# wdc3iii/legged_gym_dev

Hardware: AMD Instinct MI355X
Metric: env-steps/sec (whole node), ANYmal-C flat 4096 envs per GPU (higher is better)
Workload: dtype f32

## Files before the change

### legged_gym_dev_amd/csrc/ppo_api.hip

```cpp
#include <cstdlib>
#include <cstring>
#include <string>
#include <vector>

#include "ppo_device.h"
#include "ppo_mlp_args.h"
#include "ppo_rnn.h"

void lg_set_error(const std::string &s);

extern "C" {
void ppok_gemm_fwd(const GemmArgs *g, int nz, hipStream_t s);
void ppok_gemm_dx(const GemmArgs *g, int nz, hipStream_t s);
void ppok_sync_planes(const PpoDev *P, hipStream_t s);
int ppok_mlp_fwd(const MlpArgs *g, const PpoDev *P, hipStream_t s);
int ppok_mlp_supported(const MlpArgs *g);
int64_t ppok_mlp_frag_elems(int K, int N);
void ppok_mlp_frag_build(const MlpArgs *g, hipStream_t s);
void ppok_gemm_dw(const GemmArgs *g, int nz, hipStream_t s);
void ppok_act_sample(const PpoDev *P, const float *obs, const float *cobs, const float *mu, const float *val, int t,
                     int64_t cnt, int inject, hipStream_t s);
void ppok_process_step(const PpoDev *P, const float *rew, const uint8_t *dones, const uint8_t *tos, int t, hipStream_t s);
void ppok_gae(const PpoDev *P, const float *last_values, hipStream_t s);
void ppok_det_fold(const PpoDev *P, hipStream_t s);
void ppok_adv_normalize(const PpoDev *P, hipStream_t s);
void ppok_gather(const PpoDev *P, int mb, hipStream_t s);
void ppok_randperm(const PpoDev *P, int n, uint64_t update_idx, hipStream_t s);
void ppok_loss(const PpoDev *P, const float *mu, const float *v, float *dmu, float *dval, hipStream_t s);
// ... 61 lines not shown
    hipEvent_t ev_dz, ev_side;
    int overlap;
    long long *det_buf;
    int act_code;
    int grads_dirty;
    lg_ctx *env;
    int pp_pending, pp_t, pp_use_tos;
    int params_dirty;
    int fused_act;
    MlpArgs mlp;
    int step, inject;
    int64_t act_count, update_count;
    int Mmax;
    std::vector<void *> allocs;
    int64_t perm_count;
    struct MbSet { float *obs, *critic_obs, *actions, *mu, *scalars; } mbset[2];
    int mb_cur, mb_ready, mb_last;
    lg_ppo_buffers pub;
    Rnn rnn;
};

template <typename T>
static bool palloc(lg_ppo *p, T **out, size_t n) {
    void *q = nullptr;
    size_t bytes = (n ? n : 1) * sizeof(T);
    if (hipMalloc(&q, bytes) != hipSuccess || hipMemset(q, 0, bytes) != hipSuccess) return false;
    p->allocs.push_back(q);
    *out = (T *)q;
    return true;
}
#define PA(ptr, n) do { if (!palloc(p, &(ptr), (n))) { lg_set_error("hipMalloc failed in lg_ppo_create"); lg_ppo_destroy(p); return -100; } } while (0)
// ... 51 lines not shown
    int64_t counts[4];
    const int n = bucket_extents(p, l, bufs, counts);
    hipStream_t cs = lg_comm_stream_(p->comm);
    (void)hipEventRecord(p->ev_bucket, ready_on);
    (void)hipStreamWaitEvent(cs, p->ev_bucket, 0);
    const int rc = lg_comm_group_allreduce_(p->comm, bufs, counts, n, cs);
    if (rc && !p->comm_rc) p->comm_rc = rc;
}

static void backward(lg_ppo *p, int M, const float *in0, const float *in1, int skip_head = 0) {
    const float *in[2] = {in0, in1};
    auto det_args = [&](GemmArgs &g) {
        g.det_base = p->dev.grads; g.det64 = p->dev.det64; g.det_n = p->dev.num_params + 2;
    };
    const int nl = p->net[0].nl;
    for (int l = nl - 1 - skip_head; l >= 0; --l) {
        GemmArgs g;
        memset(&g, 0, sizeof(g));
        det_args(g);
        for (int z = 0; z < 2; ++z) {
            Net &n = p->net[z];
            g.A[z] = n.dz[l + 1]; g.lda[z] = n.dims[l + 1];
            g.B[z] = l == 0 ? in[z] : n.act[l]; g.ldb[z] = n.dims[l];
            g.C[z] = p->dev.grads + n.w_off[l]; g.ldc[z] = n.dims[l];
            g.M[z] = n.dims[l + 1]; g.N[z] = n.dims[l]; g.K[z] = M;
            if (l == 0 && !p->rnn.H) {
                const int ldp = z == 0 ? p->dev.Op : p->dev.OCp;
                g.ldb[z] = ldp;
                if (ldp != n.dims[0]) { g.N[z] = ldp; g.nstore[z] = n.dims[0]; }
            }
        }
        const bool on_side = p->overlap && l > 0;
        hipStream_t dw_stream = on_side ? p->side : p->stream;
        if (on_side) {
// ... 5 lines not shown
        if (l > 0) {
            memset(&g, 0, sizeof(g));
            det_args(g);
            for (int z = 0; z < 2; ++z) {
                Net &n = p->net[z];
                g.A[z] = n.dz[l + 1]; g.lda[z] = n.dims[l + 1];
                g.B[z] = p->dev.params + n.w_off[l]; g.ldb[z] = n.dims[l];
                g.Bpl[z] = p->dev.wpl + n.pl_off[l];
                g.C[z] = n.dz[l]; g.ldc[z] = n.dims[l];
                g.aux[z] = n.act[l]; g.ldaux[z] = n.dims[l];
                g.colsum[z] = p->dev.grads + n.b_off[l - 1];
                g.M[z] = M; g.N[z] = n.dims[l]; g.K[z] = n.dims[l + 1];
            }
            g.elu = p->act_code;
            g.pl_stride = p->dev.pl_stride;
            ppok_gemm_dx(&g, 2, p->stream);
        }
    }
    if (p->rnn.H) {
        GemmArgs g;
        memset(&g, 0, sizeof(g));
        for (int z = 0; z < 2; ++z) {
            Net &n = p->net[z];
            g.A[z] = n.dz[1]; g.lda[z] = n.dims[1];
            g.B[z] = p->dev.params + n.w_off[0]; g.ldb[z] = n.dims[0];
            g.Bpl[z] = p->dev.wpl + n.pl_off[0];
            g.C[z] = p->rnn.dh[z]; g.ldc[z] = n.dims[0];
            g.aux[z] = p->rnn.dh[z]; g.ldaux[z] = n.dims[0];
            g.M[z] = M; g.N[z] = n.dims[0]; g.K[z] = n.dims[1];
        }
        g.elu = 0;
// ... 272 lines not shown
                dest[d.seg_off[sg] + e] = (int32_t)(d.seg_pl[sg] + (e / d.seg_cols[sg]) * seg_ld[sg] + e % d.seg_cols[sg]);
        (void)hipMemcpy(d.pl_dest, dest.data(), dest.size() * sizeof(int32_t), hipMemcpyHostToDevice);
    }
    const size_t TN = (size_t)T * N;
    PA(d.st_obs, TN * O);
    if (cfg->num_critic_obs > 0) PA(d.st_critic_obs, TN * OC); else d.st_critic_obs = d.st_obs;
    PA(d.st_actions, TN * A); PA(d.st_rewards, TN); PA(d.st_values, TN); PA(d.st_returns, TN); PA(d.st_adv, TN);
    PA(d.st_log_prob, TN); PA(d.st_mu, TN * A); PA(d.st_sigma, A); PA(d.st_dones, TN);
    PA(d.act_actions, (size_t)N * A); PA(d.act_values, N); PA(d.act_log_prob, N); PA(d.act_mu, (size_t)N * A);
    PA(d.stats, 8); PA(d.loss_acc, 4 + LG_NORM_BLOCKS); PA(d.noise, (size_t)N * A); PA(d.perm, TN); PA(d.adv_partial, 4);
    for (int k = 0; k < 2; ++k) {
        lg_ppo::MbSet &m = p->mbset[k];
        PA(m.obs, (size_t)R * d.Op);
        if (cfg->num_critic_obs > 0) PA(m.critic_obs, (size_t)R * d.OCp); else m.critic_obs = m.obs;
        PA(m.actions, (size_t)R * A); PA(m.mu, (size_t)R * A); PA(m.scalars, (size_t)R * 4);
    }
    p->mb_cur = 0; p->mb_ready = -1; p->mb_last = -1;
    d.mb_obs = p->mbset[0].obs; d.mb_critic_obs = p->mbset[0].critic_obs; d.mb_actions = p->mbset[0].actions;
    d.mb_mu = p->mbset[0].mu; d.mb_scalars = p->mbset[0].scalars;
    PA(d.head_part, ppok_head_part_floats());
    PA(d.cur_reward_sum, N); PA(d.cur_episode_len, N); PA(d.ep_stats, 4); PA(d.ep_ring, 200); PA(d.ep_ring_count, 1);
    for (int z = 0; z < 2; ++z) {
        Net &n = p->net[z];
        n.act[0] = nullptr; n.dz[0] = nullptr;
        for (int l = 1; l <= n.nl; ++l) { PA(n.act[l], (size_t)p->Mmax * n.dims[l]); PA(n.dz[l], (size_t)p->Mmax * n.dims[l]); }
    }
    if (H) {
        Rnn &q = p->rnn;
        const size_t NH = (size_t)N * H, Rr = (size_t)R;
        for (int z = 0; z < 2; ++z) {
            PA(q.h[z], NH); PA(q.c[z], NH); PA(q.sv_h[z], TN * H); PA(q.sv_c[z], TN * H); PA(q.tmp_h[z], NH); PA(q.tmp_c[z], NH);
            PA(q.pg[z], Rr * 4 * H); PA(q.gates[z], Rr * 4 * H);
            PA(q.hout[z], Rr * H); PA(q.cout[z], Rr * H); PA(q.hused[z], Rr * H); PA(q.cused[z], Rr * H); PA(q.dh[z], Rr * H);
            PA(q.dc[z], (size_t)q.mbs * H);
// ... 57 lines not shown
    return 0;
}
int lg_ppo_reset_hidden(lg_ppo *p, const uint8_t *dones) {
    if (!p->rnn.H) { lg_set_error("lg_ppo_reset_hidden: not a recurrent learner"); return -15; }
    flush_rollout_epilogue(p);
    const Rnn &q = p->rnn;
    ppok_lstm_reset(q.h[0], q.c[0], q.h[1], q.c[1], dones, p->cfg.num_envs, q.H, p->stream);
    return launch_ok();
}
int lg_ppo_get_buffers(lg_ppo *p, lg_ppo_buffers *out) { *out = p->pub; return 0; }
int lg_ppo_set_stream(lg_ppo *p, void *s) { p->stream = (hipStream_t)s; return 0; }
int lg_ppo_inject_noise(lg_ppo *p, int enable) { p->inject = enable; return 0; }
int lg_ppo_debug_set_overlap(lg_ppo *p, int v) { p->overlap = v; return 0; }
int lg_ppo_debug_set_fused_act(lg_ppo *p, int v) { p->fused_act = v && p->mlp.wfrag; return 0; }
int lg_ppo_debug_get_fused_act(lg_ppo *p) { return p->fused_act; }
int lg_ppo_debug_set_act_count(lg_ppo *p, long long v) { p->act_count = v; return 0; }

int lg_ppo_param_layout(lg_ppo *p, int64_t *offsets, int64_t *shapes, int max_entries) {
    int k = 0;
    auto put = [&](int64_t o, int64_t r, int64_t c) {
        if (k < max_entries) { offsets[k] = o; shapes[2 * k] = r; shapes[2 * k + 1] = c; }
        ++k;
    };
    put(p->dev.off_std, p->cfg.num_actions, 0);
    for (int z = 0; z < 2; ++z)
        for (int l = 0; l < p->net[z].nl; ++l) {
            put(p->net[z].w_off[l], p->net[z].dims[l + 1], p->net[z].dims[l]);
            put(p->net[z].b_off[l], p->net[z].dims[l + 1], 0);
        }
    const Rnn &q = p->rnn;
// ... 119 lines not shown
    p->grads_dirty = 1;
    ppok_sync_planes(&p->dev, p->stream);
    return launch_ok();
}

int lg_ppo_minibatch_backward(lg_ppo *p, int epoch, int mb) {
    (void)epoch;
    if (rnn_update_refused(p)) return -6;
    PpoDev &d = p->dev;
    const int R = d.mb_rows;
    if (p->grads_dirty) (void)hipMemsetAsync(d.grads, 0, (size_t)(d.num_params + 2) * sizeof(float), p->stream);
    p->grads_dirty = 1;
    auto use_set = [&](PpoDev &dev, int k) {
        const lg_ppo::MbSet &m = p->mbset[k];
        dev.mb_obs = m.obs; dev.mb_critic_obs = m.critic_obs; dev.mb_actions = m.actions; dev.mb_mu = m.mu; dev.mb_scalars = m.scalars;
    };
    if (p->mb_ready == mb) {
        p->mb_cur ^= 1;
        use_set(d, p->mb_cur);
    } else {
        ppok_gather(&d, mb, p->stream);
    }
    p->mb_ready = -1;
    p->mb_last = mb;
    Net &na = p->net[0], &nc = p->net[1];
    const int nl = na.nl, H3 = na.dims[nl - 1];
    const bool fuse = p->act_code == 1 && nl >= 2 && nc.dims[nl - 1] == H3 && (H3 == 128 || H3 == 64 || H3 == 32);
    if (p->rnn.H) {
        rnn_forward_seq(p, mb);
        forward(p, R, p->rnn.hout[0], p->rnn.hout[1], 3, fuse ? 1 : 0, true, false);
// ... 11 lines not shown
        rnn_backward_seq(p, mb);
    } else
        backward(p, R, d.mb_obs, d.mb_critic_obs, fuse ? 1 : 0);
    if (d.det64) ppok_det_fold(&d, p->stream);
    if (p->comm_rc) { const int rc = p->comm_rc; p->comm_rc = 0; return rc; }
    return launch_ok();
}

int lg_ppo_minibatch_step(lg_ppo *p) {
    int next = -1;
    PpoDev other = p->dev;
    if (p->cfg.num_mini_batches > 1 && p->mb_last >= 0) {
        next = (p->mb_last + 1) % p->cfg.num_mini_batches;
        const lg_ppo::MbSet &m = p->mbset[p->mb_cur ^ 1];
        other.mb_obs = m.obs; other.mb_critic_obs = m.critic_obs; other.mb_actions = m.actions; other.mb_mu = m.mu; other.mb_scalars = m.scalars;
    }
    if (ppok_step(&p->dev, (int)(p->update_count & 1), &other, next, p->stream)) p->mb_ready = next;
    p->mb_last = -1;
    p->grads_dirty = 0;
    p->params_dirty = 1;
    p->update_count++;
    return launch_ok();
}

int lg_ppo_end_update(lg_ppo *p) { p->step = 0; return 0; }

int lg_ppo_set_comm(lg_ppo *p, lg_comm *c) {
    if (c && p->rnn.H) { lg_set_error("lg_ppo_set_comm: the per-layer gradient buckets do not cover the LSTM of a recurrent learner; reduce the whole gradient buffer between lg_ppo_minibatch_backward and lg_ppo_minibatch_step instead"); return -14; }
    if (c && p->dev.det64) { lg_set_error("gradient buckets inside the backward pass cannot be combined with deterministic mode"); return -14; }
    p->comm = c;
// ... 41 lines not shown
    const int n = bucket_extents(p, l, bufs, counts);
    for (int k = 0; k < n; ++k) offsets[k] = bufs[k] - p->dev.grads;
    return n;
}

int lg_ppo_debug_mb_sets(lg_ppo *p, void **cur, void **other, int *dims) {
    const PpoDev &d = p->dev;
    const lg_ppo::MbSet &m = p->mbset[p->mb_cur ^ 1];
    void *c[5] = {d.mb_obs, d.mb_critic_obs, d.mb_actions, d.mb_mu, d.mb_scalars};
    void *o[5] = {m.obs, m.critic_obs, m.actions, m.mu, m.scalars};
    for (int k = 0; k < 5; ++k) { cur[k] = c[k]; other[k] = o[k]; }
    dims[0] = d.Op; dims[1] = d.OCp; dims[2] = d.mb_rows;
    return 0;
}

int lg_ppo_debug_weight_planes(lg_ppo *p, void **wpl, int64_t *pl_stride, void **pl_dest) {
    if (!p || !wpl || !pl_stride || !pl_dest) { lg_set_error("null argument"); return -1; }
    *wpl = p->dev.wpl; *pl_stride = p->dev.pl_stride; *pl_dest = p->dev.pl_dest;
    return 0;
}

int lg_ppo_act_inference(lg_ppo *p, const float *obs, float *actions_out, int64_t rows) {
    if (rows > p->Mmax) { lg_set_error("too many rows for act_inference"); return -11; }
    if (p->rnn.H) {
        if (rows != p->cfg.num_envs) { lg_set_error("act_inference of a recurrent learner takes exactly num_envs rows"); return -11; }
        rnn_stash_live(p, 1, -1);
        rnn_live_step(p, 1, obs, nullptr, -1);
        obs = p->rnn.h[0];
    }
    forward(p, (int)rows, obs, nullptr, 1);
// ... 8 lines not shown
```

### legged_gym_dev_amd/csrc/ppo_device.h

```cpp
#pragma once
#include "lg_device.h"

#define LG_PPO_MAX_A 16
#define LG_PPO_MAX_LAYERS (LG_MAX_HIDDEN + 1)

struct GemmArgs {
    const float *A[2], *B[2], *bias[2], *aux[2];
    float *C[2], *colsum[2];
    int M[2], N[2], K[2], lda[2], ldb[2], ldc[2], ldaux[2];
    int elu;
    const uint16_t *Bpl[2];
    int64_t pl_stride;
    int Kpl[2], ldbpl[2];
    int nstore[2];
    const float *det_base;
    long long *det64;
    int64_t det_n;
};

#define LG_PPO_MAX_SEG (2 * LG_PPO_MAX_LAYERS)

struct PpoDev {
    int N, T, A, O, OC, mb_rows, world, env_offset;
    int adaptive, clipped_value;
    uint64_t seed;
    float gamma, lam, clip, value_coef, entropy_coef, desired_kl, max_grad_norm;
    int64_t num_params;
    int off_std, off_bias_actor_head, off_bias_critic_head;
    float *params, *grads, *adam_m, *adam_v;
    float *st_obs, *st_critic_obs, *st_actions, *st_rewards, *st_values, *st_returns, *st_adv, *st_log_prob, *st_mu, *st_sigma;
    uint8_t *st_dones;
    float *act_actions, *act_values, *act_log_prob, *act_mu;
    float *stats;
    float *loss_acc;
    float *noise;
    int32_t *perm;
    float *adv_partial;
    float *mb_obs, *mb_critic_obs, *mb_actions, *mb_mu, *mb_scalars;
    int Op, OCp;
    float *cur_reward_sum, *cur_episode_len, *ep_stats, *ep_ring;
    int32_t *ep_ring_count;
    float *head_part;
    uint16_t *wpl;
    int32_t *pl_dest;
    int64_t pl_stride;
    int nseg;
    int64_t seg_off[LG_PPO_MAX_SEG], seg_pl[LG_PPO_MAX_SEG];
    int seg_rows[LG_PPO_MAX_SEG], seg_cols[LG_PPO_MAX_SEG];
    long long *det64;
};
#define LG_DET_WORDS(num_params) ((size_t)(num_params) + 12)
#define LG_NORM_BLOCKS 128

#define LG_DET_SCALE 1099511627776.0
// ... 52 lines not shown
```

### legged_gym_dev_amd/csrc/ppo_gemm.hip

```cpp
#include <cstring>
#include <type_traits>

#include "ppo_device.h"
#include "ppo_split_bf16.h"

__device__ __forceinline__ void xcd_tile(int lin, int inner, int outer, int &o, int &i) {
    if ((outer & 7) == 0) {
        const int c = lin & 7, j = lin >> 3;
        o = c + 8 * (j / inner);
        i = j % inner;
    } else {
        o = lin / inner;
        i = lin % inner;
    }
}

#define BK 32

struct GemmTiles { int z, M, N, K, tiles_n, tiles_m; };
template <int BM, int BN>
__device__ __forceinline__ void gemm_problem(const GemmArgs &g, GemmTiles &t) {
    t.z = blockIdx.z;
    t.M = g.M[t.z]; t.N = g.N[t.z]; t.K = g.K[t.z];
    t.tiles_n = (t.N + BN - 1) / BN; t.tiles_m = (t.M + BM - 1) / BM;
// ... 609 lines not shown
            for (int d = 0; d < PD; ++d)
                if (d == 0 || k0 + d * BK < k_end)
                    body(k0 + d * BK, ra[d], rb[d], ma[d], mb[d], ra[(d + 1) % PD], rb[(d + 1) % PD], ma[(d + 1) % PD], mb[(d + 1) % PD]);
        }
    };
    if (a_vec && b_vec) run(std::true_type{});
    else run(std::false_type{});
    GEMM_EPILOGUE(2, TM, TN, BM, BN, g, z, M, g.nstore[z] ? g.nstore[z] : N, m0, n0, wm, wn, li, lk, ldc, acc);
}

static int g_gemm_x6 = 1;
extern "C" void ppok_debug_set_x6(int v) { g_gemm_x6 = v != 0; }

#include "ppo_gemm_glds.h"

struct GemmShape { int maxM, maxN; unsigned small_tiles, big_tiles; bool big; };
enum { GK_GEMM_SMALL = 1, GK_GEMM_BIG, GK_PL1_SMALL, GK_PL1_BIG, GK_PL2_SMALL, GK_PL2_BIG, GK_GLDS, GK_DW_SMALL, GK_DW_BIG, GK_REF };
struct GemmLaunch { int kernel, slices; };
static GemmShape gemm_shape(const GemmArgs &g, int nz, int splits) {
    GemmShape sh{0, 0, 0, 0, false};
    for (int z = 0; z < nz; ++z) { sh.maxM = g.M[z] > sh.maxM ? g.M[z] : sh.maxM; sh.maxN = g.N[z] > sh.maxN ? g.N[z] : sh.maxN; }
    const long big_tiles = (long)((sh.maxM + 127) / 128) * ((sh.maxN + 127) / 128);
    sh.small_tiles = (unsigned)(((sh.maxM + 63) / 64) * ((sh.maxN + 63) / 64));
    sh.big_tiles = (unsigned)big_tiles;
    sh.big = big_tiles * splits >= 192 && sh.maxN > 64 && sh.maxM > 64;
    return sh;
}

static bool planes_ok(const GemmArgs &g, int nz, int (GemmArgs::*chunked)[2]) {
    if (!g_gemm_x6) return false;
    for (int z = 0; z < nz; ++z) {
        const int d = (g.*chunked)[z];
// ... 59 lines not shown
static GemmLaunch gemm_fwd(const GemmArgs *g, int nz, hipStream_t s) {
    GemmArgs gp = *g;
    for (int z = 0; z < nz; ++z) {
        if (g->Kpl[z]) gp.K[z] = g->Kpl[z];
        if (g->ldbpl[z]) gp.ldb[z] = g->ldbpl[z];
    }
    if (planes_ok(gp, nz, &GemmArgs::K)) return launch_gemm_pl<0>(gp, nz, s);
    if (g_gemm_x6) return launch_gemm<true, true, 0>(*g, nz, s);
    return launch_gemm_ref<true, true, 0>(*g, nz, 1, s);
}
static GemmLaunch gemm_dx(const GemmArgs *g, int nz, hipStream_t s) {
    if (planes_ok(*g, nz, &GemmArgs::N)) return launch_gemm_pl<1, false, 2>(*g, nz, s);
    if (g_gemm_x6) return launch_gemm<true, false, 1>(*g, nz, s);
    return launch_gemm_ref<true, false, 1>(*g, nz, 1, s);
}
extern "C" void ppok_gemm_fwd(const GemmArgs *g, int nz, hipStream_t s) { gemm_fwd(g, nz, s); }
extern "C" void ppok_gemm_dx(const GemmArgs *g, int nz, hipStream_t s) { gemm_dx(g, nz, s); }
extern "C" void ppok_gemm_dw(const GemmArgs *g, int nz, hipStream_t s) { launch_gemm_dw(*g, nz, dw_splits(*g, nz), s); }

extern "C" int ppok_debug_gemm_args(const GemmArgs *g, int nz, int kind, int splits, void *stream, int *info) {
    if (!g || nz < 1 || nz > 2 || kind < 0 || kind > 2 || splits < 0) return -1;
    hipStream_t s = (hipStream_t)stream;
    const GemmLaunch l = kind == 0 ? gemm_fwd(g, nz, s) : kind == 1 ? gemm_dx(g, nz, s) : launch_gemm_dw(*g, nz, splits ? splits : dw_splits(*g, nz), s);
    if (info) { info[0] = l.kernel; info[1] = l.slices; }
    return 0;
}
extern "C" int ppok_debug_gemm_args_size() { return (int)sizeof(GemmArgs); }

extern "C" void ppok_debug_gemm(const float *A, const float *B, float *C, int M, int N, int K, int mode, int splits, void *stream) {
    GemmArgs g;
// ... 33 lines not shown
```

### legged_gym_dev_amd/csrc/ppo_kernels.hip

```cpp
#include <type_traits>

#include "ppo_device.h"
#include "ppo_split_bf16.h"

__global__ void k_act_sample(PpoDev P, const float *__restrict__ obs, const float *__restrict__ critic_obs,
                             const float *__restrict__ mu, const float *__restrict__ val, int t, int64_t act_count, int inject) {
    const int i = blockIdx.x * blockDim.x + threadIdx.x;
    const int N = P.N, A = P.A, O = P.O;
    if (t >= 0) {
        const size_t tot = (size_t)N * O, step = (size_t)gridDim.x * blockDim.x;
        for (size_t k = i; k < tot; k += step) P.st_obs[(size_t)t * tot + k] = obs[k];
        if (P.st_critic_obs != P.st_obs) {
            const size_t totc = (size_t)N * P.OC;
            for (size_t k = i; k < totc; k += step) P.st_critic_obs[(size_t)t * totc + k] = critic_obs[k];
        }
    }
    const float *std = P.params + P.off_std;
    if (i < A && t == 0) P.st_sigma[i] = std[i];
    if (i >= N) return;
    float lp = 0.f;
    for (int a = 0; a < A; ++a) {
        float m = mu[(size_t)i * A + a], s = std[a];
        float z = inject ? P.noise[(size_t)i * A + a] : philox_normal(P.seed, (uint32_t)(P.env_offset + i), (uint64_t)act_count, a);
        float act = m + s * z;
// ... 78 lines not shown
    for (int k = threadIdx.x; k < O; k += blockDim.x) P.mb_obs[(size_t)r * P.Op + k] = P.st_obs[(size_t)src * O + k];
    if (P.st_critic_obs != P.st_obs)
        for (int k = threadIdx.x; k < P.OC; k += blockDim.x) P.mb_critic_obs[(size_t)r * P.OCp + k] = P.st_critic_obs[(size_t)src * P.OC + k];
    if ((int)threadIdx.x < A) {
        P.mb_actions[(size_t)r * A + threadIdx.x] = P.st_actions[(size_t)src * A + threadIdx.x];
        P.mb_mu[(size_t)r * A + threadIdx.x] = P.st_mu[(size_t)src * A + threadIdx.x];
    }
    if (threadIdx.x == 0) {
        P.mb_scalars[(size_t)r * 4 + 0] = P.st_values[src];
        P.mb_scalars[(size_t)r * 4 + 1] = P.st_returns[src];
        P.mb_scalars[(size_t)r * 4 + 2] = P.st_adv[src];
        P.mb_scalars[(size_t)r * 4 + 3] = P.st_log_prob[src];
    }
}

__device__ __forceinline__ void gather4_block(const PpoDev &P, int mb, int vblock) {
    const int R = P.mb_rows, A4 = P.A / 4;
    const int gid = vblock * 256 + threadIdx.x;
    const int r = gid >> 5, j = gid & 31;
    if (r >= R) return;
    const int src = P.perm[(size_t)mb * R + r];
    const bool own_critic = P.st_critic_obs != P.st_obs;
    const int O4 = (P.O & 3) ? 0 : P.O / 4, OC4 = (own_critic && !(P.OC & 3)) ? P.OC / 4 : 0;
    auto row_copy = [&](const float *__restrict__ from, float *__restrict__ to, int n) {
        for (int k0 = j; k0 < n; k0 += 256) {
            float v[8];
#pragma unroll
            for (int u = 0; u < 8; ++u) v[u] = from[min(k0 + 32 * u, n - 1)];
#pragma unroll
            for (int u = 0; u < 8; ++u)
                if (k0 + 32 * u < n) to[k0 + 32 * u] = v[u];
        }
// ... 670 lines not shown
    (void)hipMemsetAsync(P->adv_partial, 0, 3 * sizeof(float), s);
    hipLaunchKernelGGL(k_gae, dim3((P->N + 255) / 256), dim3(256), 0, s, *P, last_values);
    if (P->det64) ppok_det_fold(P, s);
}
void ppok_adv_normalize(const PpoDev *P, hipStream_t s) {
    hipLaunchKernelGGL(k_adv_normalize, dim3(256), dim3(256), 0, s, *P);
}
void ppok_randperm(const PpoDev *P, int n, uint64_t update_idx, hipStream_t s) {
    int bits = 2;
    while ((1ll << bits) < n) ++bits;
    bits += bits & 1;
    hipLaunchKernelGGL(k_randperm, dim3((n + 255) / 256), dim3(256), 0, s, *P, n, bits / 2, update_idx);
}
void ppok_gather(const PpoDev *P, int mb, hipStream_t s) {
    if ((P->A & 3) == 0)
        hipLaunchKernelGGL(k_gather4, dim3((P->mb_rows * 32 + 255) / 256), dim3(256), 0, s, *P, mb);
    else
        hipLaunchKernelGGL(k_gather, dim3(P->mb_rows), dim3(64), 0, s, *P, mb);
}
size_t ppok_head_part_floats() { return (size_t)2 * HEAD_NET_GRID * HEAD_PART_STRIDE(128); }
int ppok_head_fused(const PpoDev *P, int H3, const float *xa, const float *xc, float *dza, float *dzc, int64_t w_a, int64_t b_a,
                    int64_t w_c, int64_t b_c, int64_t b_prev_a, int64_t b_prev_c, hipStream_t s) {
    const int ntiles = (P->mb_rows + HEAD_ROWS - 1) / HEAD_ROWS;
    dim3 grid(ntiles < HEAD_GRID ? ntiles : HEAD_GRID), block(256);
    if (H3 == 128) {
        const int nrows = ntiles < HEAD_NET_GRID ? ntiles : HEAD_NET_GRID;
        if (P->A <= 12)
            hipLaunchKernelGGL((k_head_net<128, 12>), dim3(nrows, 2), block, 0, s, *P, xa, xc, dza, dzc, P->params + w_a, P->params + w_c, b_a, b_c);
        else
            hipLaunchKernelGGL((k_head_net<128, LG_PPO_MAX_A>), dim3(nrows, 2), block, 0, s, *P, xa, xc, dza, dzc, P->params + w_a, P->params + w_c, b_a, b_c);
        constexpr int NTOT = HEAD_PART_STRIDE(128);
        hipLaunchKernelGGL((k_head_finish<128>), dim3((NTOT + 255) / 256, HEAD_FIN_CHUNKS, 2), block, 0, s, *P, nrows, w_a, b_a, w_c, b_c,
                           b_prev_a, b_prev_c);
    } else if (H3 == 64) hipLaunchKernelGGL((k_head_fused<64>), grid, block, 0, s, *P, xa, xc, dza, dzc, w_a, b_a, w_c, b_c, b_prev_a, b_prev_c);
    else if (H3 == 32) hipLaunchKernelGGL((k_head_fused<32>), grid, block, 0, s, *P, xa, xc, dza, dzc, w_a, b_a, w_c, b_c, b_prev_a, b_prev_c);
    else return -1;
    return 0;
}
void ppok_loss(const PpoDev *P, const float *mu, const float *v, float *dmu, float *dval, hipStream_t s) {
    hipLaunchKernelGGL(k_loss, dim3((P->mb_rows + 255) / 256), dim3(256), 0, s, *P, mu, v, dmu, dval);
}
void ppok_sync_planes(const PpoDev *P, hipStream_t s) { hipLaunchKernelGGL(k_sync_planes, dim3(256), dim3(256), 0, s, *P); }
int ppok_step(const PpoDev *P, int par, const PpoDev *G, int gather_mb, hipStream_t s) {
    const bool g4 = gather_mb >= 0 && (P->A & 3) == 0;
    const int gblocks = g4 ? (P->mb_rows * 32 + 255) / 256 : 0;
    hipLaunchKernelGGL(k_opt_prepare, dim3(LG_NORM_BLOCKS + gblocks), dim3(256), 0, s, *P, par, LG_NORM_BLOCKS, g4 ? *G : *P, gather_mb);
    if (P->det64) ppok_det_fold(P, s);
    constexpr int adam_max = 1024;
    const long want = (P->num_params + 255) / 256;
    hipLaunchKernelGGL(k_opt_adam, dim3((unsigned)(want < adam_max ? (want > 0 ? want : 1) : adam_max)), dim3(256), 0, s, *P, par);
    return g4 ? 1 : 0;
}
}
```

### legged_gym_dev_amd/lib.py

```python
import ctypes as C
import os
import subprocess

import numpy as np

from . import capi

_DIR = os.path.dirname(os.path.abspath(__file__))
SO_PATH = os.environ.get("LG_HIP_LIB") or os.path.join(_DIR, "lib", "liblegged_hip.so")
_lib = None


class LeggedHipError(RuntimeError):
    pass


def build(force=False):
    src = os.path.join(_DIR, "csrc")
    if force and os.path.isfile(SO_PATH):
        os.remove(SO_PATH)
    subprocess.check_call(["make", "-C", src, "-s", "-j4"])
    return SO_PATH


# ... 32 lines not shown
    lib.lg_ppo_normalize_advantages.argtypes = [vp]
    lib.lg_ppo_begin_update.argtypes = [vp]
    lib.lg_ppo_minibatch_backward.argtypes = [vp, C.c_int, C.c_int]
    lib.lg_ppo_minibatch_step.argtypes = [vp]
    lib.lg_ppo_end_update.argtypes = [vp]
    lib.lg_ppo_act_inference.argtypes = [vp, vp, vp, C.c_int64]
    lib.lg_ppo_params_changed.argtypes = [vp]
    lib.lg_ppo_set_deterministic.argtypes = [vp, C.c_int]
    lib.lg_ppo_attach_env.argtypes = [vp, vp]
    lib.lg_ppo_create_recurrent.argtypes = [C.POINTER(capi.lg_ppo_cfg), C.POINTER(capi.lg_ppo_rnn_cfg), C.POINTER(vp)]
    lib.lg_ppo_get_rnn_buffers.argtypes = [vp, C.POINTER(capi.lg_ppo_rnn_buffers)]
    lib.lg_ppo_reset_hidden.argtypes = [vp, vp]
    lib.lg_ppo_debug_bucket_extents.argtypes = [vp, C.c_int, C.POINTER(C.c_int64), C.POINTER(C.c_int64)]
    lib.lg_ppo_debug_mb_sets.argtypes = [vp, C.POINTER(vp), C.POINTER(vp), C.POINTER(C.c_int)]
    lib.lg_ppo_debug_weight_planes.argtypes = [vp, C.POINTER(vp), C.POINTER(C.c_int64), C.POINTER(vp)]


_TORCH_DT = {"f4": "float32", "u1": "uint8", "i8": "int64", "i4": "int32"}


class _DevArray:

    def __init__(self, ptr, shape, typestr, owner):
        self.__cuda_array_interface__ = {"data": (int(ptr), False), "shape": tuple(int(s) for s in shape),
                                         "typestr": typestr, "version": 2, "strides": None}
        self._owner = owner


def device_tensor(ptr, shape, dt, owner, device):
    import torch
# ... 66 lines not shown
```

### legged_gym_dev_amd/rl/ppo.py

```python
import ctypes as C
import os

import torch

from legged_gym_dev_amd import capi
from legged_gym_dev_amd.lib import LeggedHipError, device_tensor, load

_STATS = ["lr", "kl", "value_loss_sum", "surrogate_loss_sum", "adam_t", "n_updates", "adv_mean", "adv_std"]


def _vp(t):
    return C.c_void_p(t.data_ptr()) if t is not None else None


_ACTIVATIONS = {"elu": 0, "selu": 1, "relu": 2, "lrelu": 3, "tanh": 4, "sigmoid": 5, "crelu": 2}

POLICY_CLASSES = ("ActorCritic", "ActorCriticRecurrent")


def parse_policy_class(policy_class_name, policy_cfg, num_envs, num_mini_batches):
    name = policy_class_name or "ActorCritic"
    if name not in POLICY_CLASSES:
        raise NotImplementedError(f"policy_class_name {name!r}: the HIP learner implements {list(POLICY_CLASSES)}")
    if name == "ActorCritic":
# ... 214 lines not shown

    def attach_env(self, core):
        self._call("attach_env", core.ctx if core is not None else None)

    def set_deterministic(self, on=True):
        self._call("set_deterministic", 1 if on else 0)

    def debug_mb_sets(self):
        cur, other, dims = (C.c_void_p * 5)(), (C.c_void_p * 5)(), (C.c_int * 3)()
        self._call("debug_mb_sets", cur, other, dims)
        Op, OCp, R = dims[0], dims[1], dims[2]
        shapes = (("obs", (R, Op)), ("critic_obs", (R, OCp if self.privileged else Op)), ("actions", (R, self.A)), ("mu", (R, self.A)),
                  ("scalars", (R, 4)))
        return tuple({k: device_tensor(ptrs[i], s, "f4", self, self.device) for i, (k, s) in enumerate(shapes)} for ptrs in (cur, other))

    def debug_weight_planes(self):
        wpl, dest, stride = C.c_void_p(), C.c_void_p(), C.c_int64()
        self._call("debug_weight_planes", C.byref(wpl), C.byref(stride), C.byref(dest))
        n = 3 * stride.value + 8
        planes = device_tensor(wpl.value, (n // 2,), "i4", self, self.device).view(torch.bfloat16)
        return planes, device_tensor(dest.value, (self.num_params,), "i4", self, self.device), int(stride.value)

    def params_changed(self):
        self.lib.lg_ppo_params_changed(self.ctx)

    def optimizer_state_dict(self):
        from .checkpoint import adam_state_to_torch
        names = list(self.param_views.keys())
        shapes = {k: tuple(v.shape) for k, v in self.param_views.items()}
        return adam_state_to_torch(names, shapes, self.t["adam_m"][: self.num_params], self.t["adam_v"][: self.num_params],
# ... 26 lines not shown
```

Before: 7.239 million.

## Fuse first-layer weight gradient into the layer-1 dx GEMM epilogue

Adds a fused kernel that computes layer-1 input gradients and then, in the epilogue, multiplies the activated dz tile by a pre-split bf16 fragment image of the minibatch observations to accumulate the first-layer weight gradient directly. This removes the separate layer-0 dW GEMM launch and its reread of dz1 and observations. The minibatch gather kernel gains extra blocks that build the fragment images, and buffers are allocated for them. The cost is extra atomic accumulation into dW, more gather work, and extra LDS and register pressure in the dx kernel. The path is used only for non-recurrent nets with small padded obs widths.

```diff
diff --git a/legged_gym_dev_amd/csrc/ppo_api.hip b/legged_gym_dev_amd/csrc/ppo_api.hip
--- a/legged_gym_dev_amd/csrc/ppo_api.hip
+++ b/legged_gym_dev_amd/csrc/ppo_api.hip
@@ -5,6 +5,7 @@
 
 #include "ppo_device.h"
 #include "ppo_mlp_args.h"
+#include "ppo_obs_frag.h"
 #include "ppo_rnn.h"
 
 void lg_set_error(const std::string &s);
@@ -12,6 +13,7 @@
 extern "C" {
 void ppok_gemm_fwd(const GemmArgs *g, int nz, hipStream_t s);
 void ppok_gemm_dx(const GemmArgs *g, int nz, hipStream_t s);
+int ppok_gemm_dx_dw0(const GemmArgs *g, const Dw0Args *f, int nz, hipStream_t s);
 void ppok_sync_planes(const PpoDev *P, hipStream_t s);
 int ppok_mlp_fwd(const MlpArgs *g, const PpoDev *P, hipStream_t s);
 int ppok_mlp_supported(const MlpArgs *g);
@@ -103,7 +105,9 @@
     int Mmax;
     std::vector<void *> allocs;
     int64_t perm_count;
-    struct MbSet { float *obs, *critic_obs, *actions, *mu, *scalars; } mbset[2];
+    struct MbSet { float *obs, *critic_obs, *actions, *mu, *scalars; uint16_t *img, *critic_img; } mbset[2];
+    int fused_dw0;
+    int dw0_ran;
     int mb_cur, mb_ready, mb_last;
     lg_ppo_buffers pub;
     Rnn rnn;
@@ -185,10 +189,15 @@
         g.det_base = p->dev.grads; g.det64 = p->dev.det64; g.det_n = p->dev.num_params + 2;
     };
     const int nl = p->net[0].nl;
+    p->dw0_ran = 0;
     for (int l = nl - 1 - skip_head; l >= 0; --l) {
         GemmArgs g;
         memset(&g, 0, sizeof(g));
         det_args(g);
+        if (l == 0 && p->dw0_ran) {
+            if (p->comm) reduce_layer_bucket(p, 0, p->stream);
+            break;
+        }
         for (int z = 0; z < 2; ++z) {
             Net &n = p->net[z];
             g.A[z] = n.dz[l + 1]; g.lda[z] = n.dims[l + 1];
@@ -224,7 +233,15 @@
             }
             g.elu = p->act_code;
             g.pl_stride = p->dev.pl_stride;
-            ppok_gemm_dx(&g, 2, p->stream);
+            if (l == 1 && p->fused_dw0 && !p->rnn.H && in[0] == p->dev.mb_obs && in[1] == p->dev.mb_critic_obs) {
+                Dw0Args f;
+                memset(&f, 0, sizeof(f));
+                f.img[0] = p->dev.mb_img; f.img[1] = p->dev.mb_critic_img;
+                f.nob[0] = p->dev.Op / 32; f.nob[1] = p->dev.OCp / 32;
+                for (int z = 0; z < 2; ++z) { f.dw[z] = p->dev.grads + p->net[z].w_off[0]; f.ld[z] = p->net[z].dims[0]; }
+                p->dw0_ran = ppok_gemm_dx_dw0(&g, &f, 2, p->stream) != 0;
+            }
+            if (!p->dw0_ran) ppok_gemm_dx(&g, 2, p->stream);
         }
     }
     if (p->rnn.H) {
@@ -527,10 +544,18 @@
         PA(m.obs, (size_t)R * d.Op);
         if (cfg->num_critic_obs > 0) PA(m.critic_obs, (size_t)R * d.OCp); else m.critic_obs = m.obs;
         PA(m.actions, (size_t)R * A); PA(m.mu, (size_t)R * A); PA(m.scalars, (size_t)R * 4);
-    }
+        m.img = m.critic_img = nullptr;
+        if (!H && (A & 3) == 0 && d.Op <= OBS_FRAG_MAX_LD && d.OCp <= OBS_FRAG_MAX_LD) {
+            PA(m.img, (size_t)obs_frag_elems(R, d.Op));
+            if (cfg->num_critic_obs > 0) PA(m.critic_img, (size_t)obs_frag_elems(R, d.OCp)); else m.critic_img = m.img;
+        }
+    }
+    p->fused_dw0 = p->mbset[0].img != nullptr;
+    p->dw0_ran = 0;
     p->mb_cur = 0; p->mb_ready = -1; p->mb_last = -1;
     d.mb_obs = p->mbset[0].obs; d.mb_critic_obs = p->mbset[0].critic_obs; d.mb_actions = p->mbset[0].actions;
     d.mb_mu = p->mbset[0].mu; d.mb_scalars = p->mbset[0].scalars;
+    d.mb_img = p->mbset[0].img; d.mb_critic_img = p->mbset[0].critic_img;
     PA(d.head_part, ppok_head_part_floats());
     PA(d.cur_reward_sum, N); PA(d.cur_episode_len, N); PA(d.ep_stats, 4); PA(d.ep_ring, 200); PA(d.ep_ring_count, 1);
     for (int z = 0; z < 2; ++z) {
@@ -618,6 +643,8 @@
 int lg_ppo_debug_set_overlap(lg_ppo *p, int v) { p->overlap = v; return 0; }
 int lg_ppo_debug_set_fused_act(lg_ppo *p, int v) { p->fused_act = v && p->mlp.wfrag; return 0; }
 int lg_ppo_debug_get_fused_act(lg_ppo *p) { return p->fused_act; }
+int lg_ppo_debug_set_fused_dw0(lg_ppo *p, int v) { p->fused_dw0 = v && p->mbset[0].img; return 0; }
+int lg_ppo_debug_get_fused_dw0(lg_ppo *p) { return p->dw0_ran; }
 int lg_ppo_debug_set_act_count(lg_ppo *p, long long v) { p->act_count = v; return 0; }
 
 int lg_ppo_param_layout(lg_ppo *p, int64_t *offsets, int64_t *shapes, int max_entries) {
@@ -767,6 +794,7 @@
     auto use_set = [&](PpoDev &dev, int k) {
         const lg_ppo::MbSet &m = p->mbset[k];
         dev.mb_obs = m.obs; dev.mb_critic_obs = m.critic_obs; dev.mb_actions = m.actions; dev.mb_mu = m.mu; dev.mb_scalars = m.scalars;
+        dev.mb_img = m.img; dev.mb_critic_img = m.critic_img;
     };
     if (p->mb_ready == mb) {
         p->mb_cur ^= 1;
@@ -808,6 +836,7 @@
         next = (p->mb_last + 1) % p->cfg.num_mini_batches;
         const lg_ppo::MbSet &m = p->mbset[p->mb_cur ^ 1];
         other.mb_obs = m.obs; other.mb_critic_obs = m.critic_obs; other.mb_actions = m.actions; other.mb_mu = m.mu; other.mb_scalars = m.scalars;
+        other.mb_img = m.img; other.mb_critic_img = m.critic_img;
     }
     if (ppok_step(&p->dev, (int)(p->update_count & 1), &other, next, p->stream)) p->mb_ready = next;
     p->mb_last = -1;
@@ -879,6 +908,20 @@
     return 0;
 }
 
+int lg_ppo_debug_mb_images(lg_ppo *p, void **cur, void **other, int64_t *elems) {
+    const PpoDev &d = p->dev;
+    const lg_ppo::MbSet &m = p->mbset[p->mb_cur ^ 1];
+    cur[0] = d.mb_img; cur[1] = d.mb_critic_img; other[0] = m.img; other[1] = m.critic_img;
+    elems[0] = d.mb_img ? obs_frag_elems(d.mb_rows, d.Op) : 0;
+    elems[1] = d.mb_critic_img ? obs_frag_elems(d.mb_rows, d.OCp) : 0;
+    return 0;
+}
+
+int lg_ppo_debug_dz1(lg_ppo *p, void **dz, int *widths) {
+    for (int z = 0; z < 2; ++z) { dz[z] = p->net[z].dz[1]; widths[z] = p->net[z].dims[1]; }
+    return 0;
+}
+
 int lg_ppo_debug_weight_planes(lg_ppo *p, void **wpl, int64_t *pl_stride, void **pl_dest) {
     if (!p || !wpl || !pl_stride || !pl_dest) { lg_set_error("null argument"); return -1; }
     *wpl = p->dev.wpl; *pl_stride = p->dev.pl_stride; *pl_dest = p->dev.pl_dest;
diff --git a/legged_gym_dev_amd/csrc/ppo_device.h b/legged_gym_dev_amd/csrc/ppo_device.h
--- a/legged_gym_dev_amd/csrc/ppo_device.h
+++ b/legged_gym_dev_amd/csrc/ppo_device.h
@@ -16,6 +16,12 @@
     const float *det_base;
     long long *det64;
     int64_t det_n;
+};
+
+struct Dw0Args {
+    const uint16_t *img[2];
+    float *dw[2];
+    int nob[2], ld[2];
 };
 
 #define LG_PPO_MAX_SEG (2 * LG_PPO_MAX_LAYERS)
@@ -38,6 +44,7 @@
     float *adv_partial;
     float *mb_obs, *mb_critic_obs, *mb_actions, *mb_mu, *mb_scalars;
     int Op, OCp;
+    uint16_t *mb_img, *mb_critic_img;
     float *cur_reward_sum, *cur_episode_len, *ep_stats, *ep_ring;
     int32_t *ep_ring_count;
     float *head_part;
diff --git a/legged_gym_dev_amd/csrc/ppo_gemm.hip b/legged_gym_dev_amd/csrc/ppo_gemm.hip
--- a/legged_gym_dev_amd/csrc/ppo_gemm.hip
+++ b/legged_gym_dev_amd/csrc/ppo_gemm.hip
@@ -2,6 +2,7 @@
 #include <type_traits>
 
 #include "ppo_device.h"
+#include "ppo_obs_frag.h"
 #include "ppo_split_bf16.h"
 
 __device__ __forceinline__ void xcd_tile(int lin, int inner, int outer, int &o, int &i) {
@@ -647,8 +648,143 @@
 
 #include "ppo_gemm_glds.h"
 
+template <int TM, int WGN, int ACT, bool INTERIOR>
+__device__ __forceinline__ void gemm_epilogue_dw0(const GemmArgs &g, const Dw0Args &f, int z, int M, int N, int m0, int n0, int wm_v, int wn_v,
+                                                  int li, int lk, f32x16 (&acc)[TM][1], unsigned char *__restrict__ lds) {
+    constexpr int NW = 2 * WGN, RB = 2 * TM;
+    constexpr int NI = RB * 12 / NW;
+    const int wm = __builtin_amdgcn_readfirstlane(wm_v), wn = __builtin_amdgcn_readfirstlane(wn_v);
+    const int elu = g.elu;
+    const int n = n0 + wn + li, nob = f.nob[z];
+    const bool nin = INTERIOR || n < N;
+    const float *__restrict__ auxp = g.aux[z] + min(n, N - 1);
+    const int rbs = INTERIOR ? RB : min(RB, (M + 31) / 32 - m0 / 32);
+    const int nblk = rbs * 6 * nob;
+    const unsigned char *src = reinterpret_cast<const unsigned char *>(f.img[z]) + (size_t)(m0 / 32) * 6 * nob * 1024;
+    const unsigned lds0 = (unsigned)(size_t)(__attribute__((address_space(3))) unsigned char *)lds;
+    const int wave_u = __builtin_amdgcn_readfirstlane((int)threadIdx.x >> 6);
+#pragma unroll
+    for (int i = 0; i < NI; ++i) {
+        const int b = wave_u + i * NW;
+        if (b < nblk) glds16(src + (size_t)b * 1024, 16u * (threadIdx.x & 63), lds0 + b * 1024);
+    }
+    float csum = 0.f;
+#pragma unroll
+    for (int a = 0; a < TM; ++a) {
+        const int mb = m0 + wm + 32 * a + 4 * lk;
+        float aux[16];
+#pragma unroll
+        for (int r = 0; r < 16; ++r) {
+            const int m = mb + (r & 3) + 8 * (r >> 2);
+            aux[r] = auxp[(size_t)(INTERIOR ? m : min(m, M - 1)) * g.ldaux[z]];
+        }
+#pragma unroll
+        for (int r = 0; r < 16; ++r) {
+            const bool in = INTERIOR || (nin && mb + (r & 3) + 8 * (r >> 2) < M);
+            const float x = acc[a][0][r];
+            const float d = (ACT == 1 ? (aux[r] > 0.f ? 1.0f : aux[r] + 1.0f) : ACT == 0 ? 1.0f : act_bwd(elu, aux[r]));
+            acc[a][0][r] = in ? __fmul_rn(x, d) : 0.f;
+            csum = INTERIOR ? __fadd_rn(csum, acc[a][0][r]) : in ? __fmaf_rn(x, d, csum) : csum;
+        }
+    }
+    if (g.colsum[z]) {
+        csum += __shfl_xor(csum, 32);
+        if (lk == 0 && nin) acc_add(g, &g.colsum[z][n], csum);
+    }
+    asm volatile("s_waitcnt vmcnt(0)\n\ts_barrier" ::: "memory");
+    f32x16 P[2];
+#pragma unroll
+    for (int c = 0; c < 2; ++c)
+#pragma unroll
+        for (int r = 0; r < 16; ++r) P[c][r] = 0.f;
+    const uint4 *frag = reinterpret_cast<const uint4 *>(lds) + (threadIdx.x & 63);
+#pragma unroll
+    for (int a = 0; a < TM; ++a) {
+        if (!INTERIOR && m0 + wm + 32 * a >= M) continue;
+#pragma unroll
+        for (int s = 0; s < 2; ++s) {
+            bf16x8 af[3];
+            split8(make_float4(acc[a][0][8 * s], acc[a][0][8 * s + 1], acc[a][0][8 * s + 2], acc[a][0][8 * s + 3]),
+                   make_float4(acc[a][0][8 * s + 4], acc[a][0][8 * s + 5], acc[a][0][8 * s + 6], acc[a][0][8 * s + 7]), af[0], af[1], af[2]);
+#pragma unroll
+            for (int c = 0; c < 2; ++c) {
+                if (c >= nob) continue;
+                bf16x8 bf[3];
+#pragma unroll
+                for (int p = 0; p < 3; ++p)
+                    bf[p] = __builtin_bit_cast(bf16x8, frag[obs_frag_index(wm / 32 + a, s, c, p, nob, 0, 0) / 8]);
+                P[c] = mfma_x6(af, bf, P[c]);
+            }
+        }
+    }
+    __syncthreads();
+    float *slot = reinterpret_cast<float *>(lds) + (size_t)(wn / 32) * 2 * 16 * 64 + (threadIdx.x & 63);
+    if (wm) {
+#pragma unroll
+        for (int c = 0; c < 2; ++c)
+#pragma unroll
+            for (int r = 0; r < 16; ++r) slot[(c * 16 + r) * 64] = P[c][r];
+    }
+    __syncthreads();
+    if (wm) return;
+    float *__restrict__ dw = f.dw[z];
+    const int ld = f.ld[z];
+#pragma unroll
+    for (int c = 0; c < 2; ++c) {
+        if (c >= nob) continue;
+        const int o = 32 * c + li;
+#pragma unroll
+        for (int r = 0; r < 16; ++r) {
+            const int i = n0 + wn + (r & 3) + 8 * (r >> 2) + 4 * lk;
+            const float sum = P[c][r] + slot[(c * 16 + r) * 64];
+            if ((INTERIOR || i < N) && o < ld) acc_add(g, &dw[(size_t)i * ld + o], sum);
+        }
+    }
+}
+
+template <int TM, int WGN>
+__global__ void __launch_bounds__(128 * WGN, WGN == 4 ? 4 : 2) k_gemm_dx_dw0(GemmArgs g, Dw0Args f) {
+    constexpr int WGM = 2, TN = 1, BM = 32 * TM * WGM, BN = 32 * TN * WGN;
+    GemmTiles t;
+    if (!gemm_tiles<BM, BN>(g, t)) return;
+    const int z = t.z, M = t.M, N = t.N;
+    int tm, tn;
+    xcd_tile((int)blockIdx.x, t.tiles_n, t.tiles_m, tm, tn);
+    const int m0 = tm * BM, n0 = tn * BN;
+    const int k_end = t.K;
+    const float *__restrict__ A = g.A[z];
+    const int lda = g.lda[z], ldb = g.ldb[z];
+    const bool a_vec = (lda & 3) == 0 && ((uintptr_t)A & 15) == 0 && (k_end & 3) == 0 && k_end >= 4;
+    constexpr int LDS_BYTES = 3 * (x6_plane_bytes<BM>() + plt_plane_bytes<BN>());
+    static_assert(LDS_BYTES >= WGN * 2 * 16 * 64 * (int)sizeof(float) && LDS_BYTES >= BM / 32 * 12 * 1024,
+                  "the image slice and the row-wave sum of gemm_epilogue_dw0 reuse the main loop's LDS");
+    __shared__ __attribute__((aligned(1024))) unsigned char lds_raw[LDS_BYTES];
+    const int wave = threadIdx.x >> 6, lane = threadIdx.x & 63;
+    const int wm = (wave / WGN) * 32 * TM, wn = (wave % WGN) * 32 * TN;
+    const int li = lane & 31, lk = lane >> 5;
+    f32x16 acc[TM][TN];
+#pragma unroll
+    for (int a = 0; a < TM; ++a)
+#pragma unroll
+        for (int r = 0; r < 16; ++r) acc[a][0][r] = 0.f;
+    const bool fullp = a_vec && m0 + BM <= M && n0 + BN <= N && (k_end % BK) == 0;
+    if (fullp) gemm_mainloop_x6<true, false, TM, TN, WGM, WGN, true, true, 2>(A, nullptr, lda, ldb, m0, n0, M, N, 0, k_end, lds_raw, wm, wn, li, lk, acc, g.Bpl[z], g.pl_stride);
+    else if (a_vec) gemm_mainloop_x6<true, false, TM, TN, WGM, WGN, true, false, 2>(A, nullptr, lda, ldb, m0, n0, M, N, 0, k_end, lds_raw, wm, wn, li, lk, acc, g.Bpl[z], g.pl_stride);
+    else gemm_mainloop_x6<true, false, TM, TN, WGM, WGN, false, false, 2>(A, nullptr, lda, ldb, m0, n0, M, N, 0, k_end, lds_raw, wm, wn, li, lk, acc, g.Bpl[z], g.pl_stride);
+    auto epilogue = [&](auto interior) {
+        constexpr bool IN = decltype(interior)::value;
+        if (g.elu == 1) gemm_epilogue_dw0<TM, WGN, 1, IN>(g, f, z, M, N, m0, n0, wm, wn, li, lk, acc, lds_raw);
+        else if (g.elu == 0) gemm_epilogue_dw0<TM, WGN, 0, IN>(g, f, z, M, N, m0, n0, wm, wn, li, lk, acc, lds_raw);
+        else gemm_epilogue_dw0<TM, WGN, -1, IN>(g, f, z, M, N, m0, n0, wm, wn, li, lk, acc, lds_raw);
+    };
+    if (m0 + BM <= M && n0 + BN <= N) epilogue(std::true_type{});
+    else epilogue(std::false_type{});
+}
+
+
 struct GemmShape { int maxM, maxN; unsigned small_tiles, big_tiles; bool big; };
-enum { GK_GEMM_SMALL = 1, GK_GEMM_BIG, GK_PL1_SMALL, GK_PL1_BIG, GK_PL2_SMALL, GK_PL2_BIG, GK_GLDS, GK_DW_SMALL, GK_DW_BIG, GK_REF };
+enum { GK_GEMM_SMALL = 1, GK_GEMM_BIG, GK_PL1_SMALL, GK_PL1_BIG, GK_PL2_SMALL, GK_PL2_BIG, GK_GLDS, GK_DW_SMALL, GK_DW_BIG, GK_REF,
+       GK_DX_DW0_SMALL, GK_DX_DW0_BIG };
 struct GemmLaunch { int kernel, slices; };
 static GemmShape gemm_shape(const GemmArgs &g, int nz, int splits) {
     GemmShape sh{0, 0, 0, 0, false};
@@ -738,6 +874,16 @@
     if (g_gemm_x6) return launch_gemm<true, false, 1>(*g, nz, s);
     return launch_gemm_ref<true, false, 1>(*g, nz, 1, s);
 }
+static int gemm_dx_dw0(const GemmArgs *g, const Dw0Args *f, int nz, hipStream_t s) {
+    if (!planes_ok(*g, nz, &GemmArgs::N)) return 0;
+    for (int z = 0; z < nz; ++z)
+        if (!f->img[z] || !f->dw[z] || f->nob[z] < 1 || f->nob[z] > OBS_FRAG_MAX_LD / 32 || f->ld[z] > 32 * f->nob[z] || !g->aux[z]) return 0;
+    const GemmShape sh = gemm_shape(*g, nz, 1);
+    if (sh.big) hipLaunchKernelGGL((k_gemm_dx_dw0<2, 4>), dim3(sh.big_tiles, 1, nz), dim3(512), 0, s, *g, *f);
+    else hipLaunchKernelGGL((k_gemm_dx_dw0<1, 2>), dim3(sh.small_tiles, 1, nz), dim3(256), 0, s, *g, *f);
+    return sh.big ? GK_DX_DW0_BIG : GK_DX_DW0_SMALL;
+}
+extern "C" int ppok_gemm_dx_dw0(const GemmArgs *g, const Dw0Args *f, int nz, hipStream_t s) { return gemm_dx_dw0(g, f, nz, s); }
 extern "C" void ppok_gemm_fwd(const GemmArgs *g, int nz, hipStream_t s) { gemm_fwd(g, nz, s); }
 extern "C" void ppok_gemm_dx(const GemmArgs *g, int nz, hipStream_t s) { gemm_dx(g, nz, s); }
 extern "C" void ppok_gemm_dw(const GemmArgs *g, int nz, hipStream_t s) { launch_gemm_dw(*g, nz, dw_splits(*g, nz), s); }
diff --git a/legged_gym_dev_amd/csrc/ppo_kernels.hip b/legged_gym_dev_amd/csrc/ppo_kernels.hip
--- a/legged_gym_dev_amd/csrc/ppo_kernels.hip
+++ b/legged_gym_dev_amd/csrc/ppo_kernels.hip
@@ -1,6 +1,7 @@
 #include <type_traits>
 
 #include "ppo_device.h"
+#include "ppo_obs_frag.h"
 #include "ppo_split_bf16.h"
 
 __global__ void k_act_sample(PpoDev P, const float *__restrict__ obs, const float *__restrict__ critic_obs,
@@ -116,8 +117,46 @@
     }
 }
 
+__device__ __forceinline__ void gather_img_lane(const float *__restrict__ st, int W, int nob, uint16_t *__restrict__ img,
+                                                const int32_t *__restrict__ perm, int R, int task) {
+    const int lane = task & 63, t = task >> 6;
+    const int c = t % nob, s = (t / nob) & 1, rb = t / (2 * nob);
+    const int o = 32 * c + (lane & 31), kgrp = lane >> 5;
+    float v[8];
+#pragma unroll
+    for (int j = 0; j < 8; ++j) {
+        const int r = 32 * rb + obs_frag_row(s, kgrp, j);
+        const bool in = r < R && o < W;
+        const int src = perm[min(r, R - 1)];
+        const float x = st[(size_t)src * W + min(o, W - 1)];
+        v[j] = in ? x : 0.f;
+    }
+    bf16x8 pl[3];
+    split8(make_float4(v[0], v[1], v[2], v[3]), make_float4(v[4], v[5], v[6], v[7]), pl[0], pl[1], pl[2]);
+#pragma unroll
+    for (int p = 0; p < 3; ++p) *reinterpret_cast<bf16x8 *>(img + obs_frag_index(rb, s, c, p, nob, lane, 0)) = pl[p];
+}
+__host__ __device__ __forceinline__ int gather_img_tasks(int R, int ldp) { return (R + 31) / 32 * 2 * (ldp / 32) * 64; }
+__host__ __device__ __forceinline__ int gather_row_blocks(int R) { return (R * 32 + 255) / 256; }
+static int gather4_blocks(const PpoDev &P) {
+    int tasks = 0;
+    if (P.mb_img) tasks = gather_img_tasks(P.mb_rows, P.Op) + (P.mb_critic_img != P.mb_img ? gather_img_tasks(P.mb_rows, P.OCp) : 0);
+    return gather_row_blocks(P.mb_rows) + (tasks + 255) / 256;
+}
+
 __device__ __forceinline__ void gather4_block(const PpoDev &P, int mb, int vblock) {
     const int R = P.mb_rows, A4 = P.A / 4;
+    if (vblock >= gather_row_blocks(R)) {
+        if (!P.mb_img) return;
+        int task = (vblock - gather_row_blocks(R)) * 256 + threadIdx.x;
+        const int ta = gather_img_tasks(R, P.Op);
+        const int32_t *perm = P.perm + (size_t)mb * R;
+        if (task < ta) { gather_img_lane(P.st_obs, P.O, P.Op / 32, P.mb_img, perm, R, task); return; }
+        task -= ta;
+        if (P.mb_critic_img != P.mb_img && task < gather_img_tasks(R, P.OCp))
+            gather_img_lane(P.st_critic_obs, P.OC, P.OCp / 32, P.mb_critic_img, perm, R, task);
+        return;
+    }
     const int gid = vblock * 256 + threadIdx.x;
     const int r = gid >> 5, j = gid & 31;
     if (r >= R) return;
@@ -818,7 +857,7 @@
 }
 void ppok_gather(const PpoDev *P, int mb, hipStream_t s) {
     if ((P->A & 3) == 0)
-        hipLaunchKernelGGL(k_gather4, dim3((P->mb_rows * 32 + 255) / 256), dim3(256), 0, s, *P, mb);
+        hipLaunchKernelGGL(k_gather4, dim3(gather4_blocks(*P)), dim3(256), 0, s, *P, mb);
     else
         hipLaunchKernelGGL(k_gather, dim3(P->mb_rows), dim3(64), 0, s, *P, mb);
 }
@@ -847,7 +886,7 @@
 void ppok_sync_planes(const PpoDev *P, hipStream_t s) { hipLaunchKernelGGL(k_sync_planes, dim3(256), dim3(256), 0, s, *P); }
 int ppok_step(const PpoDev *P, int par, const PpoDev *G, int gather_mb, hipStream_t s) {
     const bool g4 = gather_mb >= 0 && (P->A & 3) == 0;
-    const int gblocks = g4 ? (P->mb_rows * 32 + 255) / 256 : 0;
+    const int gblocks = g4 ? gather4_blocks(*G) : 0;
     hipLaunchKernelGGL(k_opt_prepare, dim3(LG_NORM_BLOCKS + gblocks), dim3(256), 0, s, *P, par, LG_NORM_BLOCKS, g4 ? *G : *P, gather_mb);
     if (P->det64) ppok_det_fold(P, s);
     constexpr int adam_max = 1024;
diff --git a/legged_gym_dev_amd/csrc/ppo_obs_frag.h b/legged_gym_dev_amd/csrc/ppo_obs_frag.h
--- /dev/null
+++ b/legged_gym_dev_amd/csrc/ppo_obs_frag.h
@@ -0,0 +1,15 @@
+#pragma once
+#include <cstdint>
+
+#ifdef __HIPCC__
+#define OBS_FRAG_FN __host__ __device__ __forceinline__
+#else
+#define OBS_FRAG_FN inline
+#endif
+
+OBS_FRAG_FN int obs_frag_row(int s, int kgrp, int j) { return 16 * s + (j & 3) + 8 * (j >> 2) + 4 * kgrp; }
+OBS_FRAG_FN int64_t obs_frag_index(int rb, int s, int c, int plane, int nob, int lane, int j) {
+    return ((((int64_t)(2 * rb + s) * nob + c) * 3 + plane) * 64 + lane) * 8 + j;
+}
+OBS_FRAG_FN int64_t obs_frag_elems(int rows, int ldp) { return (int64_t)((rows + 31) / 32) * 2 * (ldp / 32) * 3 * 512; }
+#define OBS_FRAG_MAX_LD 64
diff --git a/legged_gym_dev_amd/lib.py b/legged_gym_dev_amd/lib.py
--- a/legged_gym_dev_amd/lib.py
+++ b/legged_gym_dev_amd/lib.py
@@ -70,6 +70,9 @@
     lib.lg_ppo_debug_bucket_extents.argtypes = [vp, C.c_int, C.POINTER(C.c_int64), C.POINTER(C.c_int64)]
     lib.lg_ppo_debug_mb_sets.argtypes = [vp, C.POINTER(vp), C.POINTER(vp), C.POINTER(C.c_int)]
     lib.lg_ppo_debug_weight_planes.argtypes = [vp, C.POINTER(vp), C.POINTER(C.c_int64), C.POINTER(vp)]
+    lib.lg_ppo_debug_mb_images.argtypes = [vp, C.POINTER(vp), C.POINTER(vp), C.POINTER(C.c_int64)]
+    lib.lg_ppo_debug_set_fused_dw0.argtypes = [vp, C.c_int]
+    lib.lg_ppo_debug_get_fused_dw0.argtypes = [vp]
 
 
 _TORCH_DT = {"f4": "float32", "u1": "uint8", "i8": "int64", "i4": "int32"}
diff --git a/legged_gym_dev_amd/rl/ppo.py b/legged_gym_dev_amd/rl/ppo.py
--- a/legged_gym_dev_amd/rl/ppo.py
+++ b/legged_gym_dev_amd/rl/ppo.py
@@ -252,6 +252,12 @@
                   ("scalars", (R, 4)))
         return tuple({k: device_tensor(ptrs[i], s, "f4", self, self.device) for i, (k, s) in enumerate(shapes)} for ptrs in (cur, other))
 
+    def debug_mb_images(self):
+        cur, other, elems = (C.c_void_p * 2)(), (C.c_void_p * 2)(), (C.c_int64 * 2)()
+        self._call("debug_mb_images", cur, other, elems)
+        view = lambda ptr, n: device_tensor(ptr, (n // 2,), "i4", self, self.device).view(torch.int16)
+        return tuple({k: view(ptrs[i], elems[i]) for i, k in enumerate(("obs", "critic_obs")) if ptrs[i]} for ptrs in (cur, other))
+
     def debug_weight_planes(self):
         wpl, dest, stride = C.c_void_p(), C.c_void_p(), C.c_int64()
         self._call("debug_weight_planes", C.byref(wpl), C.byref(stride), C.byref(dest))
```

Result: no change. 7.189 million (-0.7%).
